# jamesdolezal/biscuit

Hardware: AMD Instinct MI355X
Metric: tiles/sec at MC-dropout=30, 299x299x3 (Xception, slide-level pred/sigma reduce) (higher is better)
Workload: dtype f16; 1 GPU; BASELINE.json config 2: 1000 synthetic 299x299x3 tiles/slide, Xception f16 storage + MFMA, fp32 accumulation / BN / MC head, MC=30, batch=256, 17664 tiles/GPU resident in HBM; f16 is the 16-bit mode that holds the 1e-3 tile/slide tolerance on O(1)-logit weights (bf16, the type config 2 names, runs 5-6 % slower and misses it: bf16_value); mc_mode=head, mc_n=30, batch=256, hip_streams=1, grids_sized_for_mask=False, parallelism=slide-sharded dp1, one all-gather of slide (pred, sigma, n)

## Files before the change

### biscuit_amd/csrc/kernels_split.hip

```cpp
#include "gemm_common.h"

namespace {
using namespace bqk;

__device__ __forceinline__ unsigned relu2s(unsigned x) { return relu_pk16(x); }

template <typename T, bool RELU>
__global__ void __launch_bounds__(256) dw3x3_kernel(const T* __restrict__ in, const float* __restrict__ dw,
                                                    T* __restrict__ out, int n, int H, int W, int C) {
    if constexpr (H16<T>::F16) bq_f16_saturate();
    const int ppp = C / 8;
    const long long gid = (long long)blockIdx.x * blockDim.x + threadIdx.x;
    if (gid >= (long long)n * W * ppp) return;
    const int piece = (int)(gid % ppp);
    const int x = (int)((gid / ppp) % W);
    const int img = (int)(gid / ((long long)ppp * W));
    float w[9][8];
#pragma unroll
    for (int t = 0; t < 9; ++t) {
        const float4 a = *reinterpret_cast<const float4*>(dw + (size_t)t * C + piece * 8);
        const float4 b = *reinterpret_cast<const float4*>(dw + (size_t)t * C + piece * 8 + 4);
        w[t][0] = a.x; w[t][1] = a.y; w[t][2] = a.z; w[t][3] = a.w;
        w[t][4] = b.x; w[t][5] = b.y; w[t][6] = b.z; w[t][7] = b.w;
    }
    const T* base = in + ((size_t)img * H * W) * C + piece * 8;
    T* obase = out + ((size_t)img * H * W) * C + piece * 8;
    const bool xl = x > 0, xr = x + 1 < W;
    const uint4 zero = make_uint4(0, 0, 0, 0);
    auto load_row = [&](int y, uint4 (&r)[3]) {
        const bool vy = y >= 0 && y < H;
        const int yc = y < 0 ? 0 : (y >= H ? H - 1 : y);
        const T* p = base + ((size_t)yc * W + x) * C;
        r[1] = *reinterpret_cast<const uint4*>(p);
        r[0] = *reinterpret_cast<const uint4*>(xl ? p - C : p);
        r[2] = *reinterpret_cast<const uint4*>(xr ? p + C : p);
        if (!(vy && xl)) r[0] = zero;
        if (!vy) r[1] = zero;
        if (!(vy && xr)) r[2] = zero;
        if (RELU) {
#pragma unroll
            for (int k = 0; k < 3; ++k) {
                r[k].x = relu2s(r[k].x); r[k].y = relu2s(r[k].y); r[k].z = relu2s(r[k].z); r[k].w = relu2s(r[k].w);
            }
        }
    };
    uint4 r0[3], r1[3], r2[3];
    load_row(-1, r0);
    load_row(0, r1);
    for (int y = 0; y < H; ++y) {
        load_row(y + 1, r2);
        float acc[8];
#pragma unroll
        for (int j = 0; j < 8; ++j) acc[j] = 0.f;
#pragma unroll
        for (int dx = 0; dx < 3; ++dx) {
            float f[8];
            unpack<T>(r0[dx], f);
#pragma unroll
            for (int j = 0; j < 8; ++j) acc[j] = fmaf(w[dx][j], f[j], acc[j]);
            unpack<T>(r1[dx], f);
#pragma unroll
            for (int j = 0; j < 8; ++j) acc[j] = fmaf(w[3 + dx][j], f[j], acc[j]);
            unpack<T>(r2[dx], f);
#pragma unroll
            for (int j = 0; j < 8; ++j) acc[j] = fmaf(w[6 + dx][j], f[j], acc[j]);
        }
        *reinterpret_cast<uint4*>(obase + ((size_t)y * W + x) * C) = pack<T>(acc);
#pragma unroll
        for (int k = 0; k < 3; ++k) { r0[k] = r1[k]; r1[k] = r2[k]; }
    }
}

constexpr int BM = 128, BN = 128, BK = 64;
constexpr int A_ROW = BK * 2 + 16;
constexpr int A_BUF = BM * A_ROW;
constexpr int ST_ROW = BN * 2 + 16;

enum { EPI_PLAIN = 0, EPI_POOL = 2 };

template <typename T, int PF, bool S2, int EPI = EPI_PLAIN>
__global__ void __launch_bounds__(256) gemm_tile_kernel(const GemmParams p) {
    if constexpr (H16<T>::F16) bq_f16_saturate();
    extern __shared__ __attribute__((aligned(16))) unsigned char smem[];
    const int tid = threadIdx.x, lane = tid & 63, wave = tid >> 6;
    const int wm = wave >> 1, wn = wave & 1;
    const int r32 = lane & 31, h = lane >> 5;
    const int ntn = p.NFp / 4;
    const int tile = xcd_tile(blockIdx.x, gridDim.x);
    const int mt = tile / ntn, nt = tile - mt * ntn;
    const int m0 = mt * BM;
    const int K = p.K, KB = K / 16, NC = (K + BK - 1) / BK;
    const T* __restrict__ A = reinterpret_cast<const T*>(p.in);

    const int jp = tid & 7;
    size_t arow[4];
#pragma unroll
    for (int q = 0; q < 4; ++q) {
        int row = m0 + ((tid + q * 256) >> 3);
        row = row < p.M ? row : p.M - 1;
        if constexpr (S2) {
            const int hw = p.H * p.W;
            const int img = row / hw, rem = row - img * hw;
            const int y = rem / p.W, x = rem - y * p.W;
            arow[q] = ((size_t)(img * p.Hi + 2 * y) * p.Wi + 2 * x) * p.ldi;
        } else {
            arow[q] = (size_t)row * p.ldi;
        }
    }
    auto load_a = [&](int c, uint4 (&r)[4]) {
#pragma unroll
        for (int q = 0; q < 4; ++q) {
            const int k0 = c * BK + jp * 8;
            const int kc = k0 < K ? k0 : 0;
            uint4 v = *reinterpret_cast<const uint4*>(A + arow[q] + kc);
            if (k0 >= K) v = make_uint4(0, 0, 0, 0);
            r[q] = v;
        }
    };
    auto store_a = [&](int buf, const uint4 (&r)[4]) {
#pragma unroll
        for (int q = 0; q < 4; ++q)
            *reinterpret_cast<uint4*>(smem + buf * A_BUF + ((tid + q * 256) >> 3) * A_ROW + jp * 16) = r[q];
    };

    uint4 areg[4];
    load_a(0, areg);
    store_a(0, areg);
    load_a(1, areg);

    const int nfb = nt * 4 + wn * 2;
    const uint4* __restrict__ wp = reinterpret_cast<const uint4*>(p.wp);
    const uint4* bp0 = wp + ((size_t)nfb * p.KBtot + p.kb0) * 64 + lane;
    uint4 bq[PF][2];
#pragma unroll
    for (int d = 0; d < PF; ++d) {
        const int idx = d < KB ? d : KB - 1;
#pragma unroll
        for (int j = 0; j < 2; ++j) bq[d][j] = bp0[((size_t)j * p.KBtot + idx) * 64];
    }
    f32x16 acc[2][2];
#pragma unroll
    for (int i = 0; i < 2; ++i)
#pragma unroll
        for (int j = 0; j < 2; ++j)
#pragma unroll
            for (int e = 0; e < 16; ++e) acc[i][j][e] = 0.f;
    __syncthreads();

    for (int c = 0; c < NC; ++c) {
        const int a_base = (c & 1) * A_BUF + (wm * 64 + r32) * A_ROW + h * 16;
#pragma unroll
        for (int d = 0; d < 4; ++d) {
            const int kb = c * 4 + d;
            uint4 a[2];
#pragma unroll
            for (int i = 0; i < 2; ++i)
                a[i] = *reinterpret_cast<const uint4*>(smem + a_base + i * 32 * A_ROW + d * 32);
#pragma unroll
            for (int i = 0; i < 2; ++i)
#pragma unroll
                for (int j = 0; j < 2; ++j) mma<T>(acc[i][j], bq[d % PF][j], a[i]);
            const int nx = kb + PF;
            const int idx = nx < KB ? nx : KB - 1;
#pragma unroll
            for (int j = 0; j < 2; ++j) bq[d % PF][j] = bp0[((size_t)j * p.KBtot + idx) * 64];
        }
        if (c + 1 < NC) store_a((c + 1) & 1, areg);
        if (c + 2 < NC) load_a(c + 2, areg);
        __syncthreads();
    }

    const T* __restrict__ res = EPI == EPI_PLAIN ? reinterpret_cast<const T*>(p.residual) : nullptr;
#pragma unroll
    for (int j = 0; j < 2; ++j)
#pragma unroll
        for (int g = 0; g < 4; ++g) {
            const int nl = (wn * 2 + j) * 32 + g * 8 + h * 4;
            const int n0 = nt * BN + nl;
            float sc[4] = {1.f, 1.f, 1.f, 1.f}, bi[4] = {0.f, 0.f, 0.f, 0.f};
            if (p.scale) {
                const float4 t = *reinterpret_cast<const float4*>(p.scale + n0);
                sc[0] = t.x; sc[1] = t.y; sc[2] = t.z; sc[3] = t.w;
            }
            if (p.bias) {
                const float4 t = *reinterpret_cast<const float4*>(p.bias + n0);
                bi[0] = t.x; bi[1] = t.y; bi[2] = t.z; bi[3] = t.w;
            }
#pragma unroll
            for (int i = 0; i < 2; ++i) {
                const int rl = wm * 64 + i * 32 + r32;
                const int m = m0 + rl;
                float v[4];
#pragma unroll
                for (int e = 0; e < 4; ++e) v[e] = fmaf(acc[i][j][g * 4 + e], sc[e], bi[e]);
                if (res && m < p.M && n0 < p.Nstore) {
                    float rv[4];
                    load4<T>(res + (size_t)m * p.ldo + n0, rv);
#pragma unroll
                    for (int e = 0; e < 4; ++e) v[e] += rv[e];
                }
                if (p.relu) {
#pragma unroll
                    for (int e = 0; e < 4; ++e) v[e] = fmaxf(v[e], 0.f);
                }
                store4<T>(reinterpret_cast<T*>(smem + (size_t)rl * ST_ROW) + nl, v);
            }
        }
    __syncthreads();
    if constexpr (EPI == EPI_POOL) {
        const T* __restrict__ y = reinterpret_cast<const T*>(p.residual);
        T* __restrict__ out = reinterpret_cast<T*>(p.out);
        const int pc = tid & 15;
        const int ncol = nt * BN + pc * 8;
        const int pt = (p.Hi & 1) ? 1 : 0, pl = (p.Wi & 1) ? 1 : 0;
        if (ncol < p.Nstore) {
            const int hw = p.H * p.W;
            constexpr int RU = 2;
            for (int r0 = tid >> 4; r0 < BM; r0 += 16 * RU) {
                uint4 u[RU][9];
                int mrow[RU];
#pragma unroll
                for (int k = 0; k < RU; ++k) {
                    int m = m0 + r0 + 16 * k;
                    mrow[k] = m;
                    m = m < p.M ? m : p.M - 1;
                    const int img = m / hw, rem = m - img * hw;
                    const int yo = rem / p.W, xo = rem - yo * p.W;
#pragma unroll
                    for (int dy = 0; dy < 3; ++dy) {
                        int yy = 2 * yo + dy - pt;
                        yy = yy < 0 ? 0 : (yy > p.Hi - 1 ? p.Hi - 1 : yy);
#pragma unroll
                        for (int dx = 0; dx < 3; ++dx) {
                            int xx = 2 * xo + dx - pl;
                            xx = xx < 0 ? 0 : (xx > p.Wi - 1 ? p.Wi - 1 : xx);
                            u[k][dy * 3 + dx] = *reinterpret_cast<const uint4*>(y + ((size_t)(img * p.Hi + yy) * p.Wi + xx) * p.ldo + ncol);
                        }
                    }
                }
#pragma unroll
                for (int k = 0; k < RU; ++k) {
                    const int r = r0 + 16 * k;
                    if (r >= BM || mrow[k] >= p.M) continue;
                    float mx[8];
#pragma unroll
                    for (int j = 0; j < 8; ++j) mx[j] = -INFINITY;
#pragma unroll
                    for (int t = 0; t < 9; ++t) {
                        const T* e = reinterpret_cast<const T*>(&u[k][t]);
#pragma unroll
                        for (int j = 0; j < 8; ++j) mx[j] = fmaxf(mx[j], (float)e[j]);
                    }
                    const uint4 ru = *reinterpret_cast<const uint4*>(smem + (size_t)r * ST_ROW + pc * 16);
                    const T* re = reinterpret_cast<const T*>(&ru);
                    uint4 ou;
                    T* oe = reinterpret_cast<T*>(&ou);
#pragma unroll
                    for (int j = 0; j < 8; ++j) oe[j] = (T)(mx[j] + (float)re[j]);
                    *reinterpret_cast<uint4*>(out + (size_t)mrow[k] * p.ldo + ncol) = ou;
                }
            }
        }
    } else {
        unsigned char* __restrict__ out = reinterpret_cast<unsigned char*>(p.out);
        const int pc = tid & 15;
        const int ncol = nt * BN + pc * 8;
        if (ncol < p.Nstore) {
            for (int r = tid >> 4; r < BM; r += 16) {
                const int m = m0 + r;
                if (m < p.M)
                    *reinterpret_cast<uint4*>(out + ((size_t)m * p.ldo + ncol) * 2) =
                        *reinterpret_cast<const uint4*>(smem + (size_t)r * ST_ROW + pc * 16);
            }
        }
    }
}

}

namespace {
template <typename T>
int launch_dw3x3_t(const void* in, const float* dw, void* out, int n, int H, int W, int C, int relu, hipStream_t s) {
    const long long total = (long long)n * W * (C / 8);
    const int grid = (int)((total + 255) / 256);
    if (relu)
        hipLaunchKernelGGL((dw3x3_kernel<T, true>), dim3(grid), dim3(256), 0, s, (const T*)in, dw, (T*)out, n, H, W, C);
    else
        hipLaunchKernelGGL((dw3x3_kernel<T, false>), dim3(grid), dim3(256), 0, s, (const T*)in, dw, (T*)out, n, H, W, C);
    return (int)hipGetLastError();
}
}

int launch_dw3x3(int dtype, const void* in, const float* dw, void* out, int n, int H, int W, int C, int relu, hipStream_t s) {
    return dtype == 2 ? launch_dw3x3_t<f16_t>(in, dw, out, n, H, W, C, relu, s)
                      : launch_dw3x3_t<bf16_t>(in, dw, out, n, H, W, C, relu, s);
}

int launch_gemm_tile(int dtype, const GemmParams& p, hipStream_t s, bool pool) {
    if (p.NFp % 4 != 0 || p.K % 16 != 0 || (pool && !p.residual)) return (int)hipErrorInvalidValue;
    const size_t lds = 2 * A_BUF > BM * ST_ROW ? 2 * A_BUF : BM * ST_ROW;
    const int grid = ((p.M + BM - 1) / BM) * (p.NFp / 4);
    if (pool) {
        if (dtype == 2) hipLaunchKernelGGL((gemm_tile_kernel<f16_t, 4, true, EPI_POOL>), dim3(grid), dim3(256), lds, s, p);
        else hipLaunchKernelGGL((gemm_tile_kernel<bf16_t, 4, true, EPI_POOL>), dim3(grid), dim3(256), lds, s, p);
    } else {
        if (dtype == 2) hipLaunchKernelGGL((gemm_tile_kernel<f16_t, 4, true>), dim3(grid), dim3(256), lds, s, p);
        else hipLaunchKernelGGL((gemm_tile_kernel<bf16_t, 4, true>), dim3(grid), dim3(256), lds, s, p);
    }
    return (int)hipGetLastError();
}
```

Measured before the change: 33940 tiles/s.

## Stage depthwise 3x3 input in LDS per image slab; pipeline pool epilogue loads

The depthwise 3x3 kernel now assigns one block per (image, 32-piece channel slab). It loads the whole HxW column into LDS once, with ReLU applied on load, so the 9-tap stencil reads neighbours from LDS instead of re-reading global memory three times per row. The taps use packed half FMA helpers in place of unpack plus fmaf. Separately, the GEMM gets a min-blocks-per-CU launch bound of 3, and its pool epilogue double-buffers the 9-tap max-pool loads, issuing the first before the scale/bias epilogue. The depthwise path now rejects W>10 or LDS over 64KB, which limits it to small late-stage feature maps, and the occupancy bound may cause register spills.

```diff
diff --git a/biscuit_amd/csrc/kernels_split.hip b/biscuit_amd/csrc/kernels_split.hip
--- a/biscuit_amd/csrc/kernels_split.hip
+++ b/biscuit_amd/csrc/kernels_split.hip
@@ -5,16 +5,36 @@
 
 __device__ __forceinline__ unsigned relu2s(unsigned x) { return relu_pk16(x); }
 
+constexpr int DW_PS = 32, DW_MAXW = 10, DW_RB = 10, DW_LDS_MAX = 64 * 1024;
+
 template <typename T, bool RELU>
-__global__ void __launch_bounds__(256) dw3x3_kernel(const T* __restrict__ in, const float* __restrict__ dw,
-                                                    T* __restrict__ out, int n, int H, int W, int C) {
+__global__ void __launch_bounds__(DW_MAXW * DW_PS) dw3x3_kernel(const T* __restrict__ in, const float* __restrict__ dw,
+                                                               T* __restrict__ out, int H, int W, int C) {
     if constexpr (H16<T>::F16) bq_f16_saturate();
-    const int ppp = C / 8;
-    const long long gid = (long long)blockIdx.x * blockDim.x + threadIdx.x;
-    if (gid >= (long long)n * W * ppp) return;
-    const int piece = (int)(gid % ppp);
-    const int x = (int)((gid / ppp) % W);
-    const int img = (int)(gid / ((long long)ppp * W));
+    extern __shared__ __attribute__((aligned(16))) unsigned char smem[];
+    const int ppp = C / 8, slabs = (ppp + DW_PS - 1) / DW_PS;
+    const int img = blockIdx.x / slabs, slab = blockIdx.x - img * slabs;
+    const int pl = threadIdx.x & (DW_PS - 1), x = threadIdx.x / DW_PS;
+    const bool live = slab * DW_PS + pl < ppp;
+    const int piece = live ? slab * DW_PS + pl : ppp - 1;
+    const size_t rs = (size_t)W * C;
+    const T* base = in + ((size_t)img * H * W + x) * C + piece * 8;
+    T* obase = out + ((size_t)img * H * W + x) * C + piece * 8;
+    const int lrow = W * (DW_PS * 16);
+    unsigned char* lds = smem + x * (DW_PS * 16) + pl * 16;
+    for (int y0 = 0; y0 < H; y0 += DW_RB) {
+        uint4 col[DW_RB];
+#pragma unroll
+        for (int j = 0; j < DW_RB; ++j)
+            if (y0 + j < H) col[j] = *reinterpret_cast<const uint4*>(base + (size_t)(y0 + j) * rs);
+#pragma unroll
+        for (int j = 0; j < DW_RB; ++j)
+            if (y0 + j < H) {
+                uint4 c = col[j];
+                if (RELU) { c.x = relu2s(c.x); c.y = relu2s(c.y); c.z = relu2s(c.z); c.w = relu2s(c.w); }
+                *reinterpret_cast<uint4*>(lds + (y0 + j) * lrow) = c;
+            }
+    }
     float w[9][8];
 #pragma unroll
     for (int t = 0; t < 9; ++t) {
@@ -23,49 +43,39 @@
         w[t][0] = a.x; w[t][1] = a.y; w[t][2] = a.z; w[t][3] = a.w;
         w[t][4] = b.x; w[t][5] = b.y; w[t][6] = b.z; w[t][7] = b.w;
     }
-    const T* base = in + ((size_t)img * H * W) * C + piece * 8;
-    T* obase = out + ((size_t)img * H * W) * C + piece * 8;
+    __syncthreads();
     const bool xl = x > 0, xr = x + 1 < W;
     const uint4 zero = make_uint4(0, 0, 0, 0);
     auto load_row = [&](int y, uint4 (&r)[3]) {
-        const bool vy = y >= 0 && y < H;
-        const int yc = y < 0 ? 0 : (y >= H ? H - 1 : y);
-        const T* p = base + ((size_t)yc * W + x) * C;
-        r[1] = *reinterpret_cast<const uint4*>(p);
-        r[0] = *reinterpret_cast<const uint4*>(xl ? p - C : p);
-        r[2] = *reinterpret_cast<const uint4*>(xr ? p + C : p);
-        if (!(vy && xl)) r[0] = zero;
-        if (!vy) r[1] = zero;
-        if (!(vy && xr)) r[2] = zero;
-        if (RELU) {
-#pragma unroll
-            for (int k = 0; k < 3; ++k) {
-                r[k].x = relu2s(r[k].x); r[k].y = relu2s(r[k].y); r[k].z = relu2s(r[k].z); r[k].w = relu2s(r[k].w);
-            }
-        }
-    };
-    uint4 r0[3], r1[3], r2[3];
-    load_row(-1, r0);
+        const unsigned char* q = lds + y * lrow;
+        r[1] = *reinterpret_cast<const uint4*>(q);
+        r[0] = *reinterpret_cast<const uint4*>(xl ? q - DW_PS * 16 : q);
+        r[2] = *reinterpret_cast<const uint4*>(xr ? q + DW_PS * 16 : q);
+        if (!xl) r[0] = zero;
+        if (!xr) r[2] = zero;
+    };
+    uint4 r0[3] = {zero, zero, zero}, r1[3], r2[3];
     load_row(0, r1);
     for (int y = 0; y < H; ++y) {
-        load_row(y + 1, r2);
+        if (y + 1 < H) load_row(y + 1, r2);
+        else { r2[0] = zero; r2[1] = zero; r2[2] = zero; }
         float acc[8];
 #pragma unroll
         for (int j = 0; j < 8; ++j) acc[j] = 0.f;
+        auto tap = [&](const float (&wt)[8], const uint4& v) {
+            typedef H16<T> F;
+            acc[0] = F::fma_lo(v.x, wt[0], acc[0]); acc[1] = F::fma_hi(v.x, wt[1], acc[1]);
+            acc[2] = F::fma_lo(v.y, wt[2], acc[2]); acc[3] = F::fma_hi(v.y, wt[3], acc[3]);
+            acc[4] = F::fma_lo(v.z, wt[4], acc[4]); acc[5] = F::fma_hi(v.z, wt[5], acc[5]);
+            acc[6] = F::fma_lo(v.w, wt[6], acc[6]); acc[7] = F::fma_hi(v.w, wt[7], acc[7]);
+        };
 #pragma unroll
         for (int dx = 0; dx < 3; ++dx) {
-            float f[8];
-            unpack<T>(r0[dx], f);
-#pragma unroll
-            for (int j = 0; j < 8; ++j) acc[j] = fmaf(w[dx][j], f[j], acc[j]);
-            unpack<T>(r1[dx], f);
-#pragma unroll
-            for (int j = 0; j < 8; ++j) acc[j] = fmaf(w[3 + dx][j], f[j], acc[j]);
-            unpack<T>(r2[dx], f);
-#pragma unroll
-            for (int j = 0; j < 8; ++j) acc[j] = fmaf(w[6 + dx][j], f[j], acc[j]);
-        }
-        *reinterpret_cast<uint4*>(obase + ((size_t)y * W + x) * C) = pack<T>(acc);
+            tap(w[dx], r0[dx]);
+            tap(w[3 + dx], r1[dx]);
+            tap(w[6 + dx], r2[dx]);
+        }
+        if (live) *reinterpret_cast<uint4*>(obase + (size_t)y * rs) = pack<T>(acc);
 #pragma unroll
         for (int k = 0; k < 3; ++k) { r0[k] = r1[k]; r1[k] = r2[k]; }
     }
@@ -79,7 +89,7 @@
 enum { EPI_PLAIN = 0, EPI_POOL = 2 };
 
 template <typename T, int PF, bool S2, int EPI = EPI_PLAIN>
-__global__ void __launch_bounds__(256) gemm_tile_kernel(const GemmParams p) {
+__global__ void __launch_bounds__(256, 3) gemm_tile_kernel(const GemmParams p) {
     if constexpr (H16<T>::F16) bq_f16_saturate();
     extern __shared__ __attribute__((aligned(16))) unsigned char smem[];
     const int tid = threadIdx.x, lane = tid & 63, wave = tid >> 6;
@@ -170,6 +180,54 @@
         __syncthreads();
     }
 
+    const int pc = tid & 15;
+    const int ncol = nt * BN + pc * 8;
+    const bool col_on = ncol < p.Nstore;
+    auto pool_taps = [&](int r, uint4 (&u)[9]) {
+        const T* __restrict__ y = reinterpret_cast<const T*>(p.residual);
+        const int pt = (p.Hi & 1) ? 1 : 0, pl = (p.Wi & 1) ? 1 : 0;
+        const int hw = p.H * p.W;
+        int m = m0 + r;
+        m = m < p.M ? m : p.M - 1;
+        const int img = m / hw, rem = m - img * hw;
+        const int yo = rem / p.W, xo = rem - yo * p.W;
+#pragma unroll
+        for (int dy = 0; dy < 3; ++dy) {
+            int yy = 2 * yo + dy - pt;
+            yy = yy < 0 ? 0 : (yy > p.Hi - 1 ? p.Hi - 1 : yy);
+#pragma unroll
+            for (int dx = 0; dx < 3; ++dx) {
+                int xx = 2 * xo + dx - pl;
+                xx = xx < 0 ? 0 : (xx > p.Wi - 1 ? p.Wi - 1 : xx);
+                u[dy * 3 + dx] = *reinterpret_cast<const uint4*>(y + ((size_t)(img * p.Hi + yy) * p.Wi + xx) * p.ldo + ncol);
+            }
+        }
+    };
+    auto pool_row = [&](int r, const uint4 (&u)[9]) {
+        const int m = m0 + r;
+        if (m >= p.M) return;
+        float mx[8];
+#pragma unroll
+        for (int j = 0; j < 8; ++j) mx[j] = -INFINITY;
+#pragma unroll
+        for (int t = 0; t < 9; ++t) {
+            const T* e = reinterpret_cast<const T*>(&u[t]);
+#pragma unroll
+            for (int j = 0; j < 8; ++j) mx[j] = fmaxf(mx[j], (float)e[j]);
+        }
+        const uint4 ru = *reinterpret_cast<const uint4*>(smem + (size_t)r * ST_ROW + pc * 16);
+        const T* re = reinterpret_cast<const T*>(&ru);
+        uint4 ou;
+        T* oe = reinterpret_cast<T*>(&ou);
+#pragma unroll
+        for (int j = 0; j < 8; ++j) oe[j] = (T)(mx[j] + (float)re[j]);
+        *reinterpret_cast<uint4*>(reinterpret_cast<T*>(p.out) + (size_t)m * p.ldo + ncol) = ou;
+    };
+    uint4 ua[9], ub[9];
+    if constexpr (EPI == EPI_POOL) {
+        if (col_on) pool_taps(tid >> 4, ua);
+    }
+
     const T* __restrict__ res = EPI == EPI_PLAIN ? reinterpret_cast<const T*>(p.residual) : nullptr;
 #pragma unroll
     for (int j = 0; j < 2; ++j)
@@ -208,64 +266,19 @@
         }
     __syncthreads();
     if constexpr (EPI == EPI_POOL) {
-        const T* __restrict__ y = reinterpret_cast<const T*>(p.residual);
-        T* __restrict__ out = reinterpret_cast<T*>(p.out);
-        const int pc = tid & 15;
-        const int ncol = nt * BN + pc * 8;
-        const int pt = (p.Hi & 1) ? 1 : 0, pl = (p.Wi & 1) ? 1 : 0;
-        if (ncol < p.Nstore) {
-            const int hw = p.H * p.W;
-            constexpr int RU = 2;
-            for (int r0 = tid >> 4; r0 < BM; r0 += 16 * RU) {
-                uint4 u[RU][9];
-                int mrow[RU];
-#pragma unroll
-                for (int k = 0; k < RU; ++k) {
-                    int m = m0 + r0 + 16 * k;
-                    mrow[k] = m;
-                    m = m < p.M ? m : p.M - 1;
-                    const int img = m / hw, rem = m - img * hw;
-                    const int yo = rem / p.W, xo = rem - yo * p.W;
-#pragma unroll
-                    for (int dy = 0; dy < 3; ++dy) {
-                        int yy = 2 * yo + dy - pt;
-                        yy = yy < 0 ? 0 : (yy > p.Hi - 1 ? p.Hi - 1 : yy);
-#pragma unroll
-                        for (int dx = 0; dx < 3; ++dx) {
-                            int xx = 2 * xo + dx - pl;
-                            xx = xx < 0 ? 0 : (xx > p.Wi - 1 ? p.Wi - 1 : xx);
-                            u[k][dy * 3 + dx] = *reinterpret_cast<const uint4*>(y + ((size_t)(img * p.Hi + yy) * p.Wi + xx) * p.ldo + ncol);
-                        }
-                    }
-                }
-#pragma unroll
-                for (int k = 0; k < RU; ++k) {
-                    const int r = r0 + 16 * k;
-                    if (r >= BM || mrow[k] >= p.M) continue;
-                    float mx[8];
-#pragma unroll
-                    for (int j = 0; j < 8; ++j) mx[j] = -INFINITY;
-#pragma unroll
-                    for (int t = 0; t < 9; ++t) {
-                        const T* e = reinterpret_cast<const T*>(&u[k][t]);
-#pragma unroll
-                        for (int j = 0; j < 8; ++j) mx[j] = fmaxf(mx[j], (float)e[j]);
-                    }
-                    const uint4 ru = *reinterpret_cast<const uint4*>(smem + (size_t)r * ST_ROW + pc * 16);
-                    const T* re = reinterpret_cast<const T*>(&ru);
-                    uint4 ou;
-                    T* oe = reinterpret_cast<T*>(&ou);
-#pragma unroll
-                    for (int j = 0; j < 8; ++j) oe[j] = (T)(mx[j] + (float)re[j]);
-                    *reinterpret_cast<uint4*>(out + (size_t)mrow[k] * p.ldo + ncol) = ou;
-                }
+        if (col_on) {
+            const int r0 = tid >> 4;
+#pragma unroll
+            for (int i = 0; i < BM / 16; i += 2) {
+                pool_taps(r0 + 16 * (i + 1), ub);
+                pool_row(r0 + 16 * i, ua);
+                if (i + 2 < BM / 16) pool_taps(r0 + 16 * (i + 2), ua);
+                pool_row(r0 + 16 * (i + 1), ub);
             }
         }
     } else {
         unsigned char* __restrict__ out = reinterpret_cast<unsigned char*>(p.out);
-        const int pc = tid & 15;
-        const int ncol = nt * BN + pc * 8;
-        if (ncol < p.Nstore) {
+        if (col_on) {
             for (int r = tid >> 4; r < BM; r += 16) {
                 const int m = m0 + r;
                 if (m < p.M)
@@ -281,12 +294,15 @@
 namespace {
 template <typename T>
 int launch_dw3x3_t(const void* in, const float* dw, void* out, int n, int H, int W, int C, int relu, hipStream_t s) {
-    const long long total = (long long)n * W * (C / 8);
-    const int grid = (int)((total + 255) / 256);
+    const long long grid = (long long)n * ((C / 8 + DW_PS - 1) / DW_PS);
+    const size_t lds = (size_t)H * W * DW_PS * 16;
+    if (n <= 0 || H <= 0 || W <= 0 || W > DW_MAXW || lds > (size_t)DW_LDS_MAX || C <= 0 || C % 8 != 0 || grid > 0x7fffffffLL)
+        return (int)hipErrorInvalidValue;
+    const dim3 block(W * DW_PS);
     if (relu)
-        hipLaunchKernelGGL((dw3x3_kernel<T, true>), dim3(grid), dim3(256), 0, s, (const T*)in, dw, (T*)out, n, H, W, C);
+        hipLaunchKernelGGL((dw3x3_kernel<T, true>), dim3((unsigned)grid), block, lds, s, (const T*)in, dw, (T*)out, H, W, C);
     else
-        hipLaunchKernelGGL((dw3x3_kernel<T, false>), dim3(grid), dim3(256), 0, s, (const T*)in, dw, (T*)out, n, H, W, C);
+        hipLaunchKernelGGL((dw3x3_kernel<T, false>), dim3((unsigned)grid), block, lds, s, (const T*)in, dw, (T*)out, H, W, C);
     return (int)hipGetLastError();
 }
 }
```

Result: no change. 34030 tiles/s, median of 4 (+0.3%).
